# nv-tlabs/vid2player3d

Measured on AMD Instinct MI355X. Metric: env-steps/sec at num_envs=8192, SMPL humanoid imitation, higher is better.
Workload: dtype f32

## Files before the change

vid2player3d_amd/build.py:

```python
import os
import shutil
import subprocess
import sys

HERE = os.path.dirname(os.path.abspath(__file__))
CSRC = os.path.join(HERE, "csrc")
LIB = os.path.join(HERE, "libv2p_rollout.so")
SOURCES = ["capi.hip", "device_owner.hip", "model_compile.hip", "env.hip", "motion_state.hip", "task_ops.hip", "shape_compile.hip", "motion_build.hip", "physics.hip", "physics_ll.hip", "physics_ll_host.hip", "ball_rollout.hip", "tennis_task.hip", "mvae_player.hip", "mvae_player_dual.hip", "mvae_target.hip"]
HEADERS = ["v2p_internal.hpp", "ll_schedule.hpp", "ll_forms.hpp", "v2p_dev.hpp", "v2p_math.inc", "phys_math.hpp", "phys_common.hpp", "motion_sample.inc", "hull_gjk.hpp", "post_ops.inc", "strict_ops.inc", "tennis_task.hpp", "tennis_row.inc", "mvae_player.hpp", "mvae_player_dev.hpp", "mvae_rows.inc", "mvae_target.hpp", os.path.join("..", "..", "include", "v2p_rollout.h")]
ARCH = "gfx950"


def _hipcc():
    for c in (shutil.which("hipcc"), "/opt/rocm/bin/hipcc"):
        if c and os.path.exists(c):
            return c
    raise RuntimeError("hipcc not found: the HIP extension cannot be built")


def needs_build():
    if not os.path.exists(LIB):
        return True
    t = os.path.getmtime(LIB)
    deps = [os.path.join(CSRC, s) for s in SOURCES + HEADERS] + [os.path.abspath(__file__)]
    return any(os.path.getmtime(d) > t for d in deps)


def build_info():
    return {"arch": ARCH, "kernel_source_sha16": kernel_source_hash(), "physics_ll_math": "precise" if os.environ.get("V2P_LL_STRICT_MATH") else "relaxed (" + " ".join(LL_MATH_FLAGS) + "; precise device libraries, strict pre-physics prologue)",
            "hipcc": _hipcc()}


LL_CODEGEN_FLAGS = ["-mllvm", "-sink-insts-to-avoid-spills=1"]
LL_MATH_FLAGS = ["-fassociative-math", "-freciprocal-math", "-fno-signed-zeros", "-fno-trapping-math", "-fno-honor-nans"]
KERNEL_SOURCES = ["physics_ll.hip", "phys_common.hpp", "phys_math.hpp", "hull_gjk.hpp", "strict_ops.inc", "post_ops.inc", "v2p_math.inc", "motion_sample.inc", "v2p_internal.hpp", "ll_schedule.hpp", "ll_forms.hpp", "v2p_dev.hpp"]


def kernel_source_hash():
    import hashlib

    h = hashlib.sha256()
    for s in KERNEL_SOURCES:
        with open(os.path.join(CSRC, s), "rb") as f:
            h.update(s.encode() + b"\0" + f.read() + b"\0")
    h.update(" ".join(LL_MATH_FLAGS + LL_CODEGEN_FLAGS + [os.environ.get("V2P_LL_STRICT_MATH", ""), os.environ.get("V2P_FLAGS_PHYSICS_LL", "")]).encode())
    return h.hexdigest()[:16]


BASE_FLAGS = ["--offload-arch=" + ARCH, "-O3", "-std=c++17", "-fPIC", "-ffp-contract=fast", "-fno-vectorize", "-fno-slp-vectorize", "-Wall",
              "-Wno-unused-function"]
LL_REGS_FLAGS = ["-DV2P_LL_REGS_BUILD", "-DV2P_LL_WPS=2", "-DV2P_LL_WPS_BALL=2", "-DV2P_LL_WPS_LIMITS=2", "-DV2P_LL_PARK2=0", "-DV2P_LL_PARK3=0",
                 "-mllvm", "-amdgpu-sched-strategy=iterative-ilp"]


def compile_flags(source, regs=False):
    fl = list(BASE_FLAGS)
    if regs:
        fl += LL_REGS_FLAGS
    if source in ("motion_state.hip", "task_ops.hip", "shape_compile.hip", "motion_build.hip", "tennis_task.hip", "mvae_player.hip", "mvae_player_dual.hip", "mvae_target.hip"):
        fl = [f if f != "-ffp-contract=fast" else "-ffp-contract=off" for f in fl]
    if source in ("physics_ll.hip", "physics_ll_host.hip", "ball_rollout.hip"):
        fl = [f if f != "-ffp-contract=fast" else "-ffp-contract=fast-honor-pragmas" for f in fl]
        fl = fl + (["-DV2P_LL_STRICT_MATH"] if os.environ.get("V2P_LL_STRICT_MATH") else LL_MATH_FLAGS)
        fl = fl + LL_CODEGEN_FLAGS
    extra = os.environ.get("V2P_FLAGS_" + source.split(".")[0].upper() + ("_REGS" if regs else ""))
    if extra:
        fl = [f for f in fl if f != "-O3"] + extra.split()
    return fl


def build(force=False, verbose=False, lib_out=None, tag=""):
    if lib_out is None and not force and not needs_build():
        return LIB
    objs = []
    procs = []
    for s in SOURCES + ["physics_ll.hip:regs"]:
        regs = s.endswith(":regs")
        s = s.split(":")[0]
        obj = os.path.join(CSRC, s.replace(".hip", ("_regs" if regs else "") + tag + ".o"))
        cmd = [_hipcc()] + compile_flags(s, regs) + ["-c", os.path.join(CSRC, s), "-o", obj]
        if verbose:
            print(" ".join(cmd))
        procs.append((cmd, subprocess.Popen(cmd, stdout=subprocess.PIPE, stderr=subprocess.STDOUT)))
        objs.append(obj)
    for cmd, p in procs:
        out, _ = p.communicate()
        if p.returncode != 0:
            sys.stderr.write(out.decode())
# ... 15 lines not shown
```

vid2player3d_amd/csrc/ll_forms.hpp:

```cpp
#pragma once

namespace v2p {

enum class LlBuild { Lds, Regs };

template <LlBuild BUILD, bool TGS, bool DIAG, bool BALL, bool LIMITS>
struct LlForms {
    static constexpr bool REGS = BUILD == LlBuild::Regs;

    static constexpr bool OPAQUE_H = BALL || LIMITS;

    static constexpr bool FASTARG = REGS ? !BALL && !LIMITS && !TGS && !DIAG
                                         : !BALL && !LIMITS;

    static constexpr bool VTAB = REGS ? !LIMITS && !TGS && !BALL && !DIAG
                                      : !LIMITS && !TGS && !BALL;

    static constexpr bool SETUPX = REGS ? !LIMITS && !TGS && !BALL && !DIAG
                                        : !LIMITS && !TGS && !BALL;

    static constexpr bool LIVEM = VTAB;

    static constexpr bool ROWX = REGS ? VTAB : true;
    static constexpr bool ROWCNT = ROWX && VTAB;

    static constexpr bool UPMASK = !LIMITS && !TGS;

    static constexpr bool LAMX = true;

    static constexpr bool P2SHIFT = !(TGS && BALL);

    static constexpr bool DIAGX = REGS ? false : DIAG;

    static constexpr int waves_per_simd(int wps, int wps_ball, int wps_limits) { return DIAG ? 2 : (BALL ? wps_ball : (LIMITS ? wps_limits : wps)); }

    static_assert(SETUPX == VTAB, "the set-up in front of the sweep and the table go together");
    static_assert(LIVEM == VTAB, "the scalar live word belongs to the visit table");
    static_assert(ROWCNT == (ROWX && VTAB), "the points are counted from the visit words: no table, no count");
    static_assert(!VTAB || UPMASK, "every kernel with the visit table runs the masked way up");
};

}
```

vid2player3d_amd/csrc/physics_ll.hip:

```cpp
#include <hip/hip_runtime.h>
#include <math.h>
#include <stdlib.h>
#include <string.h>

#include <type_traits>

#if !defined(V2P_LL_STRICT_MATH)
#if !defined(V2P_LL_PRECISE_SINCOS)
#define PHYS_SINCOS(x, s, c) do { (s) = __sinf(x); (c) = __cosf(x); } while (0)
#endif
#if !defined(V2P_LL_PRECISE_SQRT)
#define PHYS_SQRT(x) __builtin_amdgcn_sqrtf(x)
#endif
#if !defined(V2P_LL_PRECISE_RCP)
#define PHYS_RCP(x) __builtin_amdgcn_rcpf(x)
#endif
#endif
#include "phys_common.hpp"
#include "hull_gjk.hpp"
#include "ll_forms.hpp"

#if defined(V2P_LL_REGS_BUILD)
#define V2P_LL_NS ll_regs
#define V2P_LL_LAUNCHER launch_env_physics_ll_regs
// ... 125 lines not shown

__device__ __forceinline__ int half_max_last(int v) {
    int o = __builtin_amdgcn_update_dpp(0, v, 0x111, 0xf, 0xf, true); v = o > v ? o : v;
    o = __builtin_amdgcn_update_dpp(0, v, 0x112, 0xf, 0xf, true); v = o > v ? o : v;
    o = __builtin_amdgcn_update_dpp(0, v, 0x114, 0xf, 0xf, true); v = o > v ? o : v;
    o = __builtin_amdgcn_update_dpp(0, v, 0x118, 0xf, 0xf, true); v = o > v ? o : v;
    o = __builtin_amdgcn_update_dpp(0, v, 0x142, 0xa, 0xf, false); v = o > v ? o : v;
    return v;
}

#define LLSAMPLED (((a.prof_heavy ? blockIdx.x < 8u : (blockIdx.x & 63) == 0)) && lane == 0)
#define LLADD(k, v) if (LLSAMPLED) atomicAdd((unsigned long long*)&a.prof[k], (unsigned long long)(v))
#define LLCOUNT(k, v) if (DIAG && a.prof && LLSAMPLED) atomicAdd((unsigned long long*)&a.prof[k], (unsigned long long)(v))
#define LLSUBV(k, tv) do { if (DIAG && a.prof) { long long t_ = clock64(); LLADD(k, t_ - tv); tv = t_; } } while (0)
#define LLSUB(k) LLSUBV(k, tsub)
#define LLSUBX(k, tv) do { if constexpr (F::DIAGX) LLSUBV(k, tv); } while (0)
#define LLSUBX_OR(k, kparent) LLSUB(F::DIAGX ? (k) : (kparent))
#define LLPH(k) LLSUBV(k, tprev)

inline namespace V2P_LL_NS {
#ifndef V2P_LL_WPS
#define V2P_LL_WPS 3
#endif
#ifndef V2P_LL_WPS_BALL
#define V2P_LL_WPS_BALL 3
#endif
#ifndef V2P_LL_WPS_LIMITS
#define V2P_LL_WPS_LIMITS 3
#endif
constexpr int LL_WPB = V2P_LL_WPB;
constexpr LlBuild LL_BUILD = V2P_LL_BUILD;
#ifndef V2P_LL_PARK2
#define V2P_LL_PARK2 1
#endif
constexpr bool PARK2 = V2P_LL_PARK2 != 0;
#ifndef V2P_LL_PARK3
#define V2P_LL_PARK3 1
#endif
constexpr bool PARK3 = V2P_LL_PARK3 != 0;
#ifndef V2P_LL_WAIT_SLEEP
#define V2P_LL_WAIT_SLEEP 16
#endif
constexpr int PARK_TAR = 0, PARK_W0 = 3, PARK_XD0 = 6, PARK_Q = 9, PARK_X = 13, PARK_CR = 16, PARK_CB = 28, PARK_CL = 32,
              PARK_SCR = PARK3 ? 44 : 16,
              PARK_SLOTS = PARK_SCR + 1;
constexpr int ROOTLAM_FLOATS = 2 * 24;
constexpr int BL_POS = 0, BL_QUAT = 3, BL_VEL = 7, BL_ANG = 10, BL_F = 13, BL_GA = 16, BL_GGAP = 17, BL_GBIAS = 18, BL_GLAM = 19, BL_GREST = 22, BL_RK = 24,
              RK_A = 0, RK_GAP = 1, RK_BIAS = 2, RK_RL = 3, RK_N = 6, RK_LAM = 9, RK_LINK = 12, RK_REST = 13, NBREC = 5, BL_V0 = BL_RK + 16 * NBREC, BL_SLOTS = BL_V0 + 8;
constexpr int ROOTLAM_ROW = ROOTLAM_FLOATS / 2, STAGE_FLOATS = NB * 13, REWARD_SLOTS = 4;
constexpr int WRENCH_FORCE_LANE = 0, WRENCH_TORQUE_LANE = 25;
constexpr int LDS_PARK = 0, LDS_STAGE = LDS_PARK, LDS_BALL = LDS_PARK + PARK_SLOTS * 64, LDS_ROOTLAM = LDS_BALL + 2 * BL_SLOTS;
constexpr int LDS_FLOATS_PER_WAVE = LDS_ROOTLAM + ROOTLAM_FLOATS;
static_assert(LDS_STAGE + 2 * STAGE_FLOATS <= LDS_BALL && REWARD_SLOTS <= PARK_SLOTS, "an overlay does not fit the parking slots");
static_assert(WRENCH_TORQUE_LANE > NB && WRENCH_TORQUE_LANE < LPE, "the torque's lane must be one without a link (and not the ball's)");
__device__ __forceinline__ void wrench_put(float* envcol, int l, float x, float y, float z) {
    envcol[l + PARK_TAR * 64] = x; envcol[l + (PARK_TAR + 1) * 64] = y; envcol[l + (PARK_TAR + 2) * 64] = z;
}
__device__ __forceinline__ float wrench_at(const float* envcol, int l, int k) { return envcol[l + (PARK_TAR + k) * 64]; }
__device__ __forceinline__ V3 wrench_get(const float* envcol, int l) { return V3{wrench_at(envcol, l, 0), wrench_at(envcol, l, 1), wrench_at(envcol, l, 2)}; }
__device__ __noinline__ f4 ball_hull_distance(ConstShape* S, int v0, int nv, V3 c) {
    V3 p;
    const float d = hull_closest([&](int k) { return V3{S->hull_verts[v0 + k][0], S->hull_verts[v0 + k][1], S->hull_verts[v0 + k][2]}; }, nv, c, p);
    return f4{p.x, p.y, p.z, d};
}
template <bool LDS>
struct ContactStore;
template <>
struct ContactStore<false> {
    V3 r_[4];
    float b_[4];
    V3 l_[4];
    __device__ __forceinline__ explicit ContactStore(float*) {}
    __device__ __forceinline__ V3 cr(int c) const { return r_[c]; }
    __device__ __forceinline__ void set_cr(int c, V3 v) { r_[c] = v; }
    __device__ __forceinline__ float bias(int c) const { return b_[c]; }
    __device__ __forceinline__ void set_bias(int c, float v) { b_[c] = v; }
    __device__ __forceinline__ V3 lam(int c) const { return l_[c]; }
    __device__ __forceinline__ void set_lam(int c, V3 v) { l_[c] = v; }
};
template <>
struct ContactStore<true> {
    float* p;
    __device__ __forceinline__ explicit ContactStore(float* park) : p(park) {}
    __device__ __forceinline__ V3 cr(int c) const { return V3{p[(PARK_CR + 3 * c) * 64], p[(PARK_CR + 3 * c + 1) * 64], p[(PARK_CR + 3 * c + 2) * 64]}; }
    __device__ __forceinline__ void set_cr(int c, V3 v) { p[(PARK_CR + 3 * c) * 64] = v.x; p[(PARK_CR + 3 * c + 1) * 64] = v.y; p[(PARK_CR + 3 * c + 2) * 64] = v.z; }
    __device__ __forceinline__ float bias(int c) const { return p[(PARK_CB + c) * 64]; }
    __device__ __forceinline__ void set_bias(int c, float v) { p[(PARK_CB + c) * 64] = v; }
    __device__ __forceinline__ V3 lam(int c) const { return V3{p[(PARK_CL + 3 * c) * 64], p[(PARK_CL + 3 * c + 1) * 64], p[(PARK_CL + 3 * c + 2) * 64]}; }
    __device__ __forceinline__ void set_lam(int c, V3 v) { p[(PARK_CL + 3 * c) * 64] = v.x; p[(PARK_CL + 3 * c + 1) * 64] = v.y; p[(PARK_CL + 3 * c + 2) * 64] = v.z; }
};

__device__ __forceinline__ void vfric_frame(const V3& w0, const V3& xd0, const V3& rr, V3& t1, V3& t2) {
    const float vx = xd0.x + w0.y * rr.z - w0.z * rr.y, vy = xd0.y + w0.z * rr.x - w0.x * rr.z;
    const float s2 = vx * vx + vy * vy;
    const bool on = s2 > 1e-12f;
    const float inv = on ? rsqrtf(s2) : 0.f;
    t1 = on ? V3{vx * inv, vy * inv, 0.f} : V3{1.f, 0.f, 0.f};
    t2 = V3{-t1.y, t1.x, 0.f};
}
template <bool CONTACT, bool MULTI, bool TGS, bool DIAG, bool BALL, bool JOBS, bool LIMITS, bool VFRIC = false>
__global__ __launch_bounds__(64 * LL_WPB, (LlForms<LL_BUILD, TGS, DIAG, BALL, LIMITS>::waves_per_simd(V2P_LL_WPS, V2P_LL_WPS_BALL, V2P_LL_WPS_LIMITS))) void physics_ll_kernel(PhysArgs a) {
    using F = LlForms<LL_BUILD, TGS, DIAG, BALL, LIMITS>;
    const int64_t N = a.n;
    const int lane = threadIdx.x & 63;
    const int half = lane >> 5;
    const int lb = lane & (LPE - 1);
// ... 391 lines not shown
                if (valid && !racket_lane) {
                    cb = mulT(R, bp - x);
                    const V3 ac{S->aabb_c[bo][0], S->aabb_c[bo][1], S->aabb_c[bo][2]}, ae{S->aabb_e[bo][0], S->aabb_e[bo][1], S->aabb_e[bo][2]};
                    const V3 ex{fmaxf(fabsf(cb.x - ac.x) - ae.x, 0.f), fmaxf(fabsf(cb.y - ac.y) - ae.y, 0.f), fmaxf(fabsf(cb.z - ac.z) - ae.z, 0.f)};
                    const V3 dv = bv0 - xd;
                    const float vmax = PHYS_SQRT(dot(dv, dv)) + PHYS_SQRT(dot(w, w)) * (PHYS_SQRT(dot(ac, ac)) + PHYS_SQRT(dot(ae, ae)));
                    const float reach = BP.radius + coff + h * vmax;
                    near = dot(ex, ex) < reach * reach && S->hull_count[bo] > 0;
                }
                if (any64(near)) {
                    float gap = 3.0e38f;
                    V3 rlw{0.f, 0.f, 0.f}, nw{0.f, 0.f, 1.f};
                    if (near) {
                        const int hv0 = S->hull_offsets[bo], hnv = S->hull_count[bo];
                        const f4 hc = ball_hull_distance(S, hv0, hnv, cb);
                        V3 pb{hc.x, hc.y, hc.z};
                        float dist = hc.w;
                        V3 nb;
                        if (dist > 1e-6f) nb = PHYS_RCP(dist) * (cb - pb);
                        else {
                            const V3 ev = cb - V3{S->aabb_c[bo][0], S->aabb_c[bo][1], S->aabb_c[bo][2]};
                            const float l = PHYS_SQRT(dot(ev, ev));
                            nb = l > 1e-5f ? PHYS_RCP(l) * ev : V3{0.f, 0.f, 1.f};
                            dist = 0.f;
                            pb = cb;
                        }
                        nw = mul(R, nb);
                        rlw = mul(R, pb);
                        const float vrel = dot(bv0 - xd - cross(w, rlw), nw);
                        const float g = dist - BP.radius;
                        if (g < coff + h * fmaxf(0.f, -vrel)) gap = g;
                    }
#pragma unroll 1
                    for (int k = 0; k < NBREC - 2; ++k) {
                        float gmin = gap;
#pragma unroll
                        for (int sh = 1; sh < 32; sh <<= 1) gmin = fminf(gmin, __shfl_xor(gmin, sh));
                        const unsigned long long wb = __ballot(gap == gmin && gap < 3.0e38f);
                        if (!wb) break;
                        const unsigned wmine = half ? (unsigned)(wb >> 32) : (unsigned)wb;
                        if (wmine && lb == __ffs(wmine) - 1) {
                            lds_vfloat* rk = bl + BL_RK + 16 * (2 + k);
                            rk[RK_A] = 1.f;
                            rk[RK_GAP] = gap;
                            rk[RK_RL] = rlw.x; rk[RK_RL + 1] = rlw.y; rk[RK_RL + 2] = rlw.z;
                            rk[RK_N] = nw.x; rk[RK_N + 1] = nw.y; rk[RK_N + 2] = nw.z;
                            rk[RK_LINK] = (float)lb;
                            gap = 3.0e38f;
                        }
                    }
                }
            }
        }
        const float mass = S->mass[bo];
        const V3 com{S->com[bo][0], S->com[bo][1], S->com[bo][2]};
        const Sym3 Ib{S->inertia[bo][0], S->inertia[bo][1], S->inertia[bo][2], S->inertia[bo][3], S->inertia[bo][4], S->inertia[bo][5]};
        V3 tau{0.f, 0.f, 0.f};
        float lsgn[3] = {0.f, 0.f, 0.f}, lbias[3] = {0.f, 0.f, 0.f}, llam[3] = {0.f, 0.f, 0.f};
        bool limact = false;
        Sym3 Kd{1.f, 0.f, 0.f, 1.f, 0.f, 1.f};
        Sym3 A;
        M3 B;
        Sym3 C{mass, 0.f, 0.f, mass, 0.f, mass};
        V3 pn, pf;
        {
            const M3 R = q2mat(q);
            const float kp = S->kp[bo], kd = S->kd[bo];
            const V3 qe = b != 0 ? quat_to_expmap_stable(jq) : V3{0.f, 0.f, 0.f};
            if (b != 0) tau = mul(R, kp * (park_get3(PARK_TAR) - qe) - (kd + h * kp) * wt);
            if (LIMITS) {
                limact = false;
                const float ih = PHYS_RCP(h);
#pragma unroll
                for (int i = 0; i < 3; ++i) {
                    const float lo = S->limit_lo[bo][i], hi = S->limit_hi[bo][i], qi = i == 0 ? qe.x : (i == 1 ? qe.y : qe.z);
                    const bool on = P.joint_limits && valid && b != 0 && hi - lo < 6.28f;
                    const float clo = qi - lo, chi = hi - qi;
                    const float gap = clo <= chi ? clo : chi;
                    lsgn[i] = on ? (clo <= chi ? 1.f : -1.f) : 0.f;
                    lbias[i] = TGS ? gap : (gap >= 0.f ? gap * ih : fmaxf(P.erp * gap * ih, -P.max_depen));
                    llam[i] = 0.f;
                    limact = limact || on;
                }
            }
            V3 dc = mul(R, com);
            V3 k0 = mul(Ib, V3{R.m[0], R.m[1], R.m[2]});
            V3 k1 = mul(Ib, V3{R.m[3], R.m[4], R.m[5]});
            V3 k2 = mul(Ib, V3{R.m[6], R.m[7], R.m[8]});
            V3 r0 = row(R, 0), r1 = row(R, 1), r2 = row(R, 2);
            Sym3 Ic{dot(r0, k0), dot(r0, k1), dot(r0, k2), dot(r1, k1), dot(r1, k2), dot(r2, k2)};
            float dd = dot(dc, dc);
            A = Sym3{Ic.xx + mass * (dd - dc.x * dc.x), Ic.xy - mass * dc.x * dc.y, Ic.xz - mass * dc.x * dc.z,
                     Ic.yy + mass * (dd - dc.y * dc.y), Ic.yz - mass * dc.y * dc.z, Ic.zz + mass * (dd - dc.z * dc.z)};
            B.m[0] = 0.f;            B.m[1] = -mass * dc.z;  B.m[2] = mass * dc.y;
            B.m[3] = mass * dc.z;    B.m[4] = 0.f;           B.m[5] = -mass * dc.x;
            B.m[6] = -mass * dc.y;   B.m[7] = mass * dc.x;   B.m[8] = 0.f;
            V3 wwd = cross(w, cross(w, dc));
            pf = mass * (wwd - V3{0.f, 0.f, P.gravity_z});
            pn = cross(w, mul(Ic, w)) + cross(dc, pf);
            if (b == 0 && wrench_on) {
                V3 extF, extT;
                if (a.actions) {
                    extF = wrench_get(wrench_park, WRENCH_FORCE_LANE);
                    extT = wrench_get(wrench_park, WRENCH_TORQUE_LANE);
                } else {
                    const float* cw = a.ctrl + env_here() * CTRL_SLOTS;
// ... 82 lines not shown
                }
            }
        }

        LLPH(PROF_PASS2);
        unpark_vel(w, xd);
        Blocks Lam;
        Lam.A = Lam.C = Sym3{1.f, 0.f, 0.f, 1.f, 0.f, 1.f};
#pragma unroll
        for (int i = 0; i < 9; ++i) Lam.B.m[i] = 0.f;
        V3 al{0.f, 0.f, 0.f}, ac{0.f, 0.f, 0.f}, dw{0.f, 0.f, 0.f}, dv{0.f, 0.f, 0.f};
        if (lb == 0) {
            float a6[21], inv6[21];
            a6[tri(0, 0)] = A.xx; a6[tri(1, 0)] = A.xy; a6[tri(2, 0)] = A.xz; a6[tri(1, 1)] = A.yy; a6[tri(2, 1)] = A.yz; a6[tri(2, 2)] = A.zz;
#pragma unroll
            for (int i = 0; i < 3; ++i)
#pragma unroll
                for (int j = 0; j < 3; ++j) a6[tri(3 + i, j)] = B.m[3 * j + i];
            a6[tri(3, 3)] = C.xx; a6[tri(4, 3)] = C.xy; a6[tri(5, 3)] = C.xz; a6[tri(4, 4)] = C.yy; a6[tri(5, 4)] = C.yz; a6[tri(5, 5)] = C.zz;
            spd6_inverse(a6, inv6);
            Lam.A = Sym3{inv6[tri(0, 0)], inv6[tri(1, 0)], inv6[tri(2, 0)], inv6[tri(1, 1)], inv6[tri(2, 1)], inv6[tri(2, 2)]};
#pragma unroll
            for (int i = 0; i < 3; ++i)
#pragma unroll
                for (int j = 0; j < 3; ++j) Lam.B.m[3 * i + j] = inv6[tri(3 + j, i)];
            Lam.C = Sym3{inv6[tri(3, 3)], inv6[tri(4, 3)], inv6[tri(5, 3)], inv6[tri(4, 4)], inv6[tri(5, 4)], inv6[tri(5, 5)]};
            al = -(mul(Lam.A, pn) + mul(Lam.B, pf));
            ac = -(V3{dot(col(Lam.B, 0), pn), dot(col(Lam.B, 1), pn), dot(col(Lam.B, 2), pn)} + mul(Lam.C, pf));
            dw = h * al;
            dv = h * ac;
            w = w + dw;
            xd = xd + dv;
        }

        for (int d = 1; d <= maxd; ++d) {
            const bool nc = (nonchain >> d) & 1;
            V3 alp = pp(al, nc), acp = pp(ac, nc), dwp = pp(dw, nc), dvp = pp(dv, nc);
            if (dep == d) {
                V3 aw = alp + zw;
                V3 av = acp + cross(alp, r) + zv;
                V3 qdd = mul(Di, u + aug * aw) - aw - mul(E, av);
                al = aw + qdd;
                ac = av;
                dw = dwp + h * qdd;
                dv = dvp + cross(dwp, r);
                w = w + dw;
                xd = xd + dv;
            }
        }

        LLPH(PROF_PASS3);
        if (CONTACT) park_vel(w, xd);
        float* const rootlam = wave_lds + LDS_ROOTLAM + half * ROOTLAM_ROW;
        if (PARK2 && CONTACT && lb == 0) {
            const float lv[21] = {Lam.A.xx, Lam.A.xy, Lam.A.xz, Lam.A.yy, Lam.A.yz, Lam.A.zz, Lam.B.m[0], Lam.B.m[1], Lam.B.m[2], Lam.B.m[3], Lam.B.m[4], Lam.B.m[5],
                                  Lam.B.m[6], Lam.B.m[7], Lam.B.m[8], Lam.C.xx, Lam.C.xy, Lam.C.xz, Lam.C.yy, Lam.C.yz, Lam.C.zz};
#pragma unroll
            for (int k = 0; k < 21; ++k) rootlam[k] = lv[k];
        }
        if (PARK2 && CONTACT) {
            Lam.A = Lam.C = Sym3{1.f, 0.f, 0.f, 1.f, 0.f, 1.f};
#pragma unroll
            for (int i = 0; i < 9; ++i) Lam.B.m[i] = 0.f;
        }
        q = Q4{park[PARK_Q * 64], park[(PARK_Q + 1) * 64], park[(PARK_Q + 2) * 64], park[(PARK_Q + 3) * 64]};
        x = park_get3(PARK_X);
        int cnt = 0;
        ContactStore<PARK3> CS(park);
#pragma unroll
        for (int c = 0; c < 4; ++c) { CS.set_cr(c, V3{0.f, 0.f, 0.f}); CS.set_bias(c, 0.f); CS.set_lam(c, V3{0.f, 0.f, 0.f}); }
        if (CONTACT) {
            const float coff = P.contact_offset;
            const int v0 = S->hull_offsets[bo], nv = S->hull_count[bo];
            const float rz0 = 2.f * (q.x * q.z - q.w * q.y), rz1 = 2.f * (q.y * q.z + q.w * q.x), rz2 = 1.f - 2.f * (q.x * q.x + q.y * q.y);
            const float zlow = x.z + rz0 * S->aabb_c[bo][0] + rz1 * S->aabb_c[bo][1] + rz2 * S->aabb_c[bo][2] -
                               (fabsf(rz0) * S->aabb_e[bo][0] + fabsf(rz1) * S->aabb_e[bo][1] + fabsf(rz2) * S->aabb_e[bo][2]);
            const bool near = valid && (zlow < coff + 1e-4f);
            int pack = 0x0fffffff;
            long long tsub = DIAG && a.prof ? clock64() : 0;
            const unsigned long long nball = __ballot(near);
            LLSUB(PROF_CULL);
            if (nball) {
                const unsigned nm = half ? (unsigned)(nball >> 32) : (unsigned)nball;
                const int nr0 = __popc((unsigned)nball), nr1 = __popc((unsigned)(nball >> 32));
                const int ntot = nr0 + nr1;
                const int rounds = (ntot + 7) >> 3;
                const int myk = (half ? nr0 : 0) + __popc(nm & ((1u << lb) - 1u));
                const int grp = lane >> 3, gl = lane & 7;
                int* const scr = (int*)(wave_lds + LDS_PARK + PARK_SCR * 64);
                if (near) scr[myk] = lane;
                LLCOUNT(PROF_ROUNDS, rounds);
                for (int rd = 0; rd < rounds; ++rd) {
                    const int kk = 8 * rd + grp;
                    const bool gon = kk < ntot;
                    const int src = gon ? scr[kk] : lane;
                    const M3 RL = q2mat(pull(q, src));
                    const V3 xL = pull(x, src);
                    const float r6 = RL.m[6], r7 = RL.m[7], r8 = RL.m[8], xz = xL.z;
                    const int v0L = __builtin_amdgcn_ds_bpermute(src << 2, v0), nvL = __builtin_amdgcn_ds_bpermute(src << 2, nv);
                    ConstShape* const SL = MULTI ? (ConstShape*)(a.shapes + __builtin_amdgcn_ds_bpermute(src << 2, sid)) : S;
                    auto hullv = [&](int idx) -> float4 { return make_float4(SL->hull_verts[idx][0], SL->hull_verts[idx][1], SL->hull_verts[idx][2], 0.f); };
                    const float r0 = RL.m[0], r1 = RL.m[1], r2 = RL.m[2], xx = xL.x;
                    const float r3 = RL.m[3], r4 = RL.m[4], r5 = RL.m[5], xy = xL.y;
                    const unsigned gbit = 1u << gl;
                    float4 vv[8];
#pragma unroll
                    for (int k = 0; k < 8; ++k) {
                        const int i = 8 * k + gl;
                        vv[k] = hullv(v0L + ((gon && i < nvL) ? i : 0));
                    }
                    float px[8], py[8];
                    unsigned clo = 0u, chi = 0u;
                    int k0 = -1;
                    float zmin = 0.f;
#pragma unroll
                    for (int k = 0; k < 8; ++k) {
                        const int i = 8 * k + gl;
                        const bool in = gon && i < nvL;
                        const float z = xz + r6 * vv[k].x + r7 * vv[k].y + r8 * vv[k].z;
                        px[k] = xx + r0 * vv[k].x + r1 * vv[k].y + r2 * vv[k].z;
                        py[k] = xy + r3 * vv[k].x + r4 * vv[k].y + r5 * vv[k].z;
                        const bool c = in && (z < coff);
                        const unsigned bit = c ? gbit << (8 * (k & 3)) : 0u;
                        if (k < 4) clo |= bit; else chi |= bit;
                        const bool better = c && (k0 < 0 || z < zmin);
                        k0 = better ? i : k0;
                        zmin = better ? z : zmin;
                    }
                    clo |= grp_xor1(clo); chi |= grp_xor1(chi);
                    clo |= grp_xor2(clo); chi |= grp_xor2(chi);
                    clo |= grp_mirror(clo); chi |= grp_mirror(chi);
                    grp_arg<false, F::FASTARG>(zmin, k0);
                    const unsigned long long cm = ((unsigned long long)chi << 32) | clo;
                    const int cntg = __popc(clo) + __popc(chi);
                    unsigned long long t = cm;
                    int s0 = t ? __ffsll((long long)t) - 1 : -1; t &= t - 1;
                    int s1 = t ? __ffsll((long long)t) - 1 : -1; t &= t - 1;
                    int s2 = t ? __ffsll((long long)t) - 1 : -1; t &= t - 1;
                    int s3 = t ? __ffsll((long long)t) - 1 : -1;
                    int ns = cntg < 4 ? cntg : 4;
                    const bool big = gon && cntg > 4;
                    if (any64(big)) {
                        LLCOUNT(PROF_MANIFOLDS, 1ull);
                        const int k0s = k0 < 0 ? 0 : k0;
                        const float4 u0 = hullv(v0L + k0s);
                        const float p0x = xx + r0 * u0.x + r1 * u0.y + r2 * u0.z;
                        const float p0y = xy + r3 * u0.x + r4 * u0.y + r5 * u0.z;
                        const unsigned long long remB = big ? (cm & ~(1ull << k0s)) : 0ull;
                        const unsigned blo = (unsigned)remB, bhi = (unsigned)(remB >> 32);
                        int k1 = -1;
                        float best = -1.f;
#pragma unroll
                        for (int k = 0; k < 8; ++k) {
                            const bool on = ((k < 4 ? blo : bhi) & (gbit << (8 * (k & 3)))) != 0u;
                            const float dx = px[k] - p0x, dy = py[k] - p0y;
                            const float d2 = dx * dx + dy * dy;
                            const bool take = on && (d2 > best);
                            best = take ? d2 : best;
                            k1 = take ? 8 * k + gl : k1;
                        }
                        grp_arg<true, F::FASTARG>(best, k1);
                        const int k1s = k1 < 0 ? 0 : k1;
                        const float4 u1 = hullv(v0L + k1s);
                        const float ex = xx + r0 * u1.x + r1 * u1.y + r2 * u1.z - p0x;
                        const float ey = xy + r3 * u1.x + r4 * u1.y + r5 * u1.z - p0y;
                        const unsigned long long remC = remB & ~(1ull << k1s);
                        const unsigned elo = (unsigned)remC, ehi = (unsigned)(remC >> 32);
                        int k2 = -1, k3 = -1;
                        float amax = 0.f, amin = 0.f;
#pragma unroll
                        for (int k = 0; k < 8; ++k) {
                            const bool on = ((k < 4 ? elo : ehi) & (gbit << (8 * (k & 3)))) != 0u;
                            const float dx = px[k] - p0x, dy = py[k] - p0y;
                            const float area = ex * dy - ey * dx;
                            const bool up = on && area > amax;
                            const bool dn = on && area < amin;
                            amax = up ? area : amax; k2 = up ? 8 * k + gl : k2;
                            amin = dn ? area : amin; k3 = dn ? 8 * k + gl : k3;
                        }
                        grp_arg<true, F::FASTARG>(amax, k2);
                        grp_arg<false, F::FASTARG>(amin, k3);
                        if (big) {
                            s0 = k0; s1 = k1;
                            s2 = k2 >= 0 ? k2 : k3;
                            s3 = k2 >= 0 ? k3 : -1;
                            ns = 2 + (k2 >= 0 ? 1 : 0) + (k3 >= 0 ? 1 : 0);
                        }
                    }
                    const int gpack = (s0 & 0x7f) | ((s1 & 0x7f) << 7) | ((s2 & 0x7f) << 14) | ((s3 & 0x7f) << 21) | (ns << 28);
                    const int got = __builtin_amdgcn_ds_bpermute(((myk & 7) << 3) << 2, gpack);
                    pack = (near && (myk >> 3) == rd) ? got : pack;
                }
            }
            LLSUB(PROF_SCAN);
            int sel4[4];
#pragma unroll
            for (int c = 0; c < 4; ++c) {
                const int sv = (pack >> (7 * c)) & 0x7f;
                sel4[c] = sv == 0x7f ? -1 : sv;
            }
            cnt = (pack >> 28) & 7;
            if (any64(cnt > 0)) {
                const M3 R = q2mat(q);
                const float ih = 1.f / h;
#pragma unroll
                for (int c = 0; c < 4; ++c) {
                    const float4 uu = hullv(v0 + (sel4[c] < 0 ? 0 : sel4[c]));
                    const V3 crc = mul(R, V3{uu.x, uu.y, uu.z});
                    CS.set_cr(c, crc);
                    float dz = x.z + crc.z - P.rest_offset;
                    CS.set_bias(c, TGS ? dz : (dz >= 0.f ? dz * ih : fmaxf(P.erp * dz * ih, -P.max_depen)));
                }
            }
            if (a.contact_ids && last && valid && live_env && !frozen) {
#pragma unroll
                for (int c = 0; c < 4; ++c) a.contact_ids[(env_here() * NB + b) * 4 + c] = c < cnt ? b * 64 + sel4[c] : -1;
            }
            if (a.contact_ids_sub && valid && live_env && !frozen) {
#pragma unroll
                for (int c = 0; c < 4; ++c) a.contact_ids_sub[((env_here() * nsub + sub) * NB + b) * 4 + c] = c < cnt ? b * 64 + sel4[c] : -1;
            }

            LLSUB(PROF_POINTS);
            if (PARK2 && lb == 0) {
                float lv[21];
#pragma unroll
                for (int k = 0; k < 21; ++k) lv[k] = rootlam[k];
                Lam.A = Sym3{lv[0], lv[1], lv[2], lv[3], lv[4], lv[5]};
#pragma unroll
                for (int k = 0; k < 9; ++k) Lam.B.m[k] = lv[6 + k];
                Lam.C = Sym3{lv[15], lv[16], lv[17], lv[18], lv[19], lv[20]};
            }
            auto ball_rec_mine = [&](int j) -> bool { return j < 2 ? racket_lane : lb == (int)bl[BL_RK + 16 * j + RK_LINK]; };
            bool myhull = false;
            if (BALL) {
#pragma unroll
                for (int j = 2; j < NBREC; ++j) myhull = myhull || (bl[BL_RK + 16 * j + RK_A] != 0.f && lb == (int)bl[BL_RK + 16 * j + RK_LINK]);
            }
            const bool ballhit = BALL && valid && ((racket_lane && (bl[BL_RK + RK_A] != 0.f || bl[BL_RK + 16 + RK_A] != 0.f)) || myhull);
            const bool ballground = BALL && ball_lane && bl[BL_GA] != 0.f;
            const bool touched = valid && (cnt > 0 || ballhit);
            const unsigned long long tb = __ballot(touched);
            const unsigned m0 = (unsigned)tb, m1 = (unsigned)(tb >> 32);
            if (LIMITS && any64(limact)) {
                const V3 wv = PARK2 ? park_get3(PARK_W0) : w;
                const V3 pwv = pp(wv, true);
                const V3 om = mulT(q2mat(q), wv - pwv);
                const float mrate = P.limit_margin * PHYS_RCP(h);
                const float lscale = TGS ? PHYS_RCP(h) : 1.f;
                bool anyrow = false;
#pragma unroll
                for (int i = 0; i < 3; ++i) {
                    const float omi = i == 0 ? om.x : (i == 1 ? om.y : om.z);
                    const bool on = lsgn[i] != 0.f && lbias[i] * lscale < mrate + fmaxf(0.f, -lsgn[i] * omi);
                    if (!on) lsgn[i] = 0.f;
                    anyrow = anyrow || on;
                }
                limact = anyrow;
            }
            const unsigned long long lmb = LIMITS ? __ballot(valid && limact) : 0ull;
            const unsigned lm0 = (unsigned)lmb, lm1 = (unsigned)(lmb >> 32);
            if (DIAG && a.wave_times) { const int tt = __popc(half ? m1 : m0); tsum += tt; tmaxs = tt > tmaxs ? tt : tmaxs; }
            [[maybe_unused]] int tdep0 = 0, tdep1 = 0;
            if constexpr (F::SETUPX) {
                const int tdred = half_max_last(touched ? dep : 0);
                tdep0 = __builtin_amdgcn_readlane(tdred, 31);
                tdep1 = __builtin_amdgcn_readlane(tdred, 63);
            }
            if (last) {
                const unsigned mine = half ? m1 : m0;
                ksum = __popc(mine);
                if constexpr (F::SETUPX) {
                    kdep = half ? tdep1 : tdep0;
                } else {
                    kdep = 0;
                    for (unsigned t = mine; t; t &= t - 1) { const int dd = M.depth[__ffs(t) - 1]; kdep = dd > kdep ? dd : kdep; }
                }
// ... 1052 lines not shown
```

Measured before the change: 23.89 million.

## Generate contacts before the articulated passes in visit-table kernels

Moves contact generation (hull culling, vertex scan, manifold selection) into a shared include and, for kernel forms that use the visit table, runs it right after the pose is known instead of after pass 3. This avoids parking and reloading q, x and the root Lambda through LDS around the contact scan. It also shifts register pressure, since the contact store is now live across the mass-matrix passes. A static assert is added to check that the parking slots used by the passes do not overlap the contact records or the scratch row.

```diff
diff --git a/vid2player3d_amd/build.py b/vid2player3d_amd/build.py
--- a/vid2player3d_amd/build.py
+++ b/vid2player3d_amd/build.py
@@ -7,7 +7,7 @@
 CSRC = os.path.join(HERE, "csrc")
 LIB = os.path.join(HERE, "libv2p_rollout.so")
 SOURCES = ["capi.hip", "device_owner.hip", "model_compile.hip", "env.hip", "motion_state.hip", "task_ops.hip", "shape_compile.hip", "motion_build.hip", "physics.hip", "physics_ll.hip", "physics_ll_host.hip", "ball_rollout.hip", "tennis_task.hip", "mvae_player.hip", "mvae_player_dual.hip", "mvae_target.hip"]
-HEADERS = ["v2p_internal.hpp", "ll_schedule.hpp", "ll_forms.hpp", "v2p_dev.hpp", "v2p_math.inc", "phys_math.hpp", "phys_common.hpp", "motion_sample.inc", "hull_gjk.hpp", "post_ops.inc", "strict_ops.inc", "tennis_task.hpp", "tennis_row.inc", "mvae_player.hpp", "mvae_player_dev.hpp", "mvae_rows.inc", "mvae_target.hpp", os.path.join("..", "..", "include", "v2p_rollout.h")]
+HEADERS = ["v2p_internal.hpp", "ll_schedule.hpp", "ll_forms.hpp", "ll_contact_setup.inc", "v2p_dev.hpp", "v2p_math.inc", "phys_math.hpp", "phys_common.hpp", "motion_sample.inc", "hull_gjk.hpp", "post_ops.inc", "strict_ops.inc", "tennis_task.hpp", "tennis_row.inc", "mvae_player.hpp", "mvae_player_dev.hpp", "mvae_rows.inc", "mvae_target.hpp", os.path.join("..", "..", "include", "v2p_rollout.h")]
 ARCH = "gfx950"
 
 
@@ -33,7 +33,7 @@
 
 LL_CODEGEN_FLAGS = ["-mllvm", "-sink-insts-to-avoid-spills=1"]
 LL_MATH_FLAGS = ["-fassociative-math", "-freciprocal-math", "-fno-signed-zeros", "-fno-trapping-math", "-fno-honor-nans"]
-KERNEL_SOURCES = ["physics_ll.hip", "phys_common.hpp", "phys_math.hpp", "hull_gjk.hpp", "strict_ops.inc", "post_ops.inc", "v2p_math.inc", "motion_sample.inc", "v2p_internal.hpp", "ll_schedule.hpp", "ll_forms.hpp", "v2p_dev.hpp"]
+KERNEL_SOURCES = ["physics_ll.hip", "phys_common.hpp", "phys_math.hpp", "hull_gjk.hpp", "strict_ops.inc", "post_ops.inc", "v2p_math.inc", "motion_sample.inc", "v2p_internal.hpp", "ll_schedule.hpp", "ll_forms.hpp", "ll_contact_setup.inc", "v2p_dev.hpp"]
 
 
 def kernel_source_hash():
diff --git a/vid2player3d_amd/csrc/ll_contact_setup.inc b/vid2player3d_amd/csrc/ll_contact_setup.inc
--- /dev/null
+++ b/vid2player3d_amd/csrc/ll_contact_setup.inc
@@ -0,0 +1,156 @@
+#pragma unroll
+for (int c = 0; c < 4; ++c) { CS.set_cr(c, V3{0.f, 0.f, 0.f}); CS.set_bias(c, 0.f); CS.set_lam(c, V3{0.f, 0.f, 0.f}); }
+if (CONTACT) {
+    const float coff = P.contact_offset;
+    const int v0 = S->hull_offsets[bo], nv = S->hull_count[bo];
+    const float rz0 = 2.f * (q.x * q.z - q.w * q.y), rz1 = 2.f * (q.y * q.z + q.w * q.x), rz2 = 1.f - 2.f * (q.x * q.x + q.y * q.y);
+    const float zlow = x.z + rz0 * S->aabb_c[bo][0] + rz1 * S->aabb_c[bo][1] + rz2 * S->aabb_c[bo][2] -
+                       (fabsf(rz0) * S->aabb_e[bo][0] + fabsf(rz1) * S->aabb_e[bo][1] + fabsf(rz2) * S->aabb_e[bo][2]);
+    const bool near = valid && (zlow < coff + 1e-4f);
+    int pack = 0x0fffffff;
+    long long tsub = DIAG && a.prof ? clock64() : 0;
+    const unsigned long long nball = __ballot(near);
+    LLSUB(PROF_CULL);
+    if (nball) {
+        const unsigned nm = half ? (unsigned)(nball >> 32) : (unsigned)nball;
+        const int nr0 = __popc((unsigned)nball), nr1 = __popc((unsigned)(nball >> 32));
+        const int ntot = nr0 + nr1;
+        const int rounds = (ntot + 7) >> 3;
+        const int myk = (half ? nr0 : 0) + __popc(nm & ((1u << lb) - 1u));
+        const int grp = lane >> 3, gl = lane & 7;
+        int* const scr = (int*)(wave_lds + LDS_PARK + PARK_SCR * 64);
+        if (near) scr[myk] = lane;
+        LLCOUNT(PROF_ROUNDS, rounds);
+        for (int rd = 0; rd < rounds; ++rd) {
+            const int kk = 8 * rd + grp;
+            const bool gon = kk < ntot;
+            const int src = gon ? scr[kk] : lane;
+            const M3 RL = q2mat(pull(q, src));
+            const V3 xL = pull(x, src);
+            const float r6 = RL.m[6], r7 = RL.m[7], r8 = RL.m[8], xz = xL.z;
+            const int v0L = __builtin_amdgcn_ds_bpermute(src << 2, v0), nvL = __builtin_amdgcn_ds_bpermute(src << 2, nv);
+            ConstShape* const SL = MULTI ? (ConstShape*)(a.shapes + __builtin_amdgcn_ds_bpermute(src << 2, sid)) : S;
+            auto hullv = [&](int idx) -> float4 { return make_float4(SL->hull_verts[idx][0], SL->hull_verts[idx][1], SL->hull_verts[idx][2], 0.f); };
+            const float r0 = RL.m[0], r1 = RL.m[1], r2 = RL.m[2], xx = xL.x;
+            const float r3 = RL.m[3], r4 = RL.m[4], r5 = RL.m[5], xy = xL.y;
+            const unsigned gbit = 1u << gl;
+            float4 vv[8];
+#pragma unroll
+            for (int k = 0; k < 8; ++k) {
+                const int i = 8 * k + gl;
+                vv[k] = hullv(v0L + ((gon && i < nvL) ? i : 0));
+            }
+            float px[8], py[8];
+            unsigned clo = 0u, chi = 0u;
+            int k0 = -1;
+            float zmin = 0.f;
+#pragma unroll
+            for (int k = 0; k < 8; ++k) {
+                const int i = 8 * k + gl;
+                const bool in = gon && i < nvL;
+                const float z = xz + r6 * vv[k].x + r7 * vv[k].y + r8 * vv[k].z;
+                px[k] = xx + r0 * vv[k].x + r1 * vv[k].y + r2 * vv[k].z;
+                py[k] = xy + r3 * vv[k].x + r4 * vv[k].y + r5 * vv[k].z;
+                const bool c = in && (z < coff);
+                const unsigned bit = c ? gbit << (8 * (k & 3)) : 0u;
+                if (k < 4) clo |= bit; else chi |= bit;
+                const bool better = c && (k0 < 0 || z < zmin);
+                k0 = better ? i : k0;
+                zmin = better ? z : zmin;
+            }
+            clo |= grp_xor1(clo); chi |= grp_xor1(chi);
+            clo |= grp_xor2(clo); chi |= grp_xor2(chi);
+            clo |= grp_mirror(clo); chi |= grp_mirror(chi);
+            grp_arg<false, F::FASTARG>(zmin, k0);
+            const unsigned long long cm = ((unsigned long long)chi << 32) | clo;
+            const int cntg = __popc(clo) + __popc(chi);
+            unsigned long long t = cm;
+            int s0 = t ? __ffsll((long long)t) - 1 : -1; t &= t - 1;
+            int s1 = t ? __ffsll((long long)t) - 1 : -1; t &= t - 1;
+            int s2 = t ? __ffsll((long long)t) - 1 : -1; t &= t - 1;
+            int s3 = t ? __ffsll((long long)t) - 1 : -1;
+            int ns = cntg < 4 ? cntg : 4;
+            const bool big = gon && cntg > 4;
+            if (any64(big)) {
+                LLCOUNT(PROF_MANIFOLDS, 1ull);
+                const int k0s = k0 < 0 ? 0 : k0;
+                const float4 u0 = hullv(v0L + k0s);
+                const float p0x = xx + r0 * u0.x + r1 * u0.y + r2 * u0.z;
+                const float p0y = xy + r3 * u0.x + r4 * u0.y + r5 * u0.z;
+                const unsigned long long remB = big ? (cm & ~(1ull << k0s)) : 0ull;
+                const unsigned blo = (unsigned)remB, bhi = (unsigned)(remB >> 32);
+                int k1 = -1;
+                float best = -1.f;
+#pragma unroll
+                for (int k = 0; k < 8; ++k) {
+                    const bool on = ((k < 4 ? blo : bhi) & (gbit << (8 * (k & 3)))) != 0u;
+                    const float dx = px[k] - p0x, dy = py[k] - p0y;
+                    const float d2 = dx * dx + dy * dy;
+                    const bool take = on && (d2 > best);
+                    best = take ? d2 : best;
+                    k1 = take ? 8 * k + gl : k1;
+                }
+                grp_arg<true, F::FASTARG>(best, k1);
+                const int k1s = k1 < 0 ? 0 : k1;
+                const float4 u1 = hullv(v0L + k1s);
+                const float ex = xx + r0 * u1.x + r1 * u1.y + r2 * u1.z - p0x;
+                const float ey = xy + r3 * u1.x + r4 * u1.y + r5 * u1.z - p0y;
+                const unsigned long long remC = remB & ~(1ull << k1s);
+                const unsigned elo = (unsigned)remC, ehi = (unsigned)(remC >> 32);
+                int k2 = -1, k3 = -1;
+                float amax = 0.f, amin = 0.f;
+#pragma unroll
+                for (int k = 0; k < 8; ++k) {
+                    const bool on = ((k < 4 ? elo : ehi) & (gbit << (8 * (k & 3)))) != 0u;
+                    const float dx = px[k] - p0x, dy = py[k] - p0y;
+                    const float area = ex * dy - ey * dx;
+                    const bool up = on && area > amax;
+                    const bool dn = on && area < amin;
+                    amax = up ? area : amax; k2 = up ? 8 * k + gl : k2;
+                    amin = dn ? area : amin; k3 = dn ? 8 * k + gl : k3;
+                }
+                grp_arg<true, F::FASTARG>(amax, k2);
+                grp_arg<false, F::FASTARG>(amin, k3);
+                if (big) {
+                    s0 = k0; s1 = k1;
+                    s2 = k2 >= 0 ? k2 : k3;
+                    s3 = k2 >= 0 ? k3 : -1;
+                    ns = 2 + (k2 >= 0 ? 1 : 0) + (k3 >= 0 ? 1 : 0);
+                }
+            }
+            const int gpack = (s0 & 0x7f) | ((s1 & 0x7f) << 7) | ((s2 & 0x7f) << 14) | ((s3 & 0x7f) << 21) | (ns << 28);
+            const int got = __builtin_amdgcn_ds_bpermute(((myk & 7) << 3) << 2, gpack);
+            pack = (near && (myk >> 3) == rd) ? got : pack;
+        }
+    }
+    LLSUB(PROF_SCAN);
+    int sel4[4];
+#pragma unroll
+    for (int c = 0; c < 4; ++c) {
+        const int sv = (pack >> (7 * c)) & 0x7f;
+        sel4[c] = sv == 0x7f ? -1 : sv;
+    }
+    cnt = (pack >> 28) & 7;
+    if (any64(cnt > 0)) {
+        const M3 R = q2mat(q);
+        const float ih = 1.f / h;
+#pragma unroll
+        for (int c = 0; c < 4; ++c) {
+            const float4 uu = hullv(v0 + (sel4[c] < 0 ? 0 : sel4[c]));
+            const V3 crc = mul(R, V3{uu.x, uu.y, uu.z});
+            CS.set_cr(c, crc);
+            float dz = x.z + crc.z - P.rest_offset;
+            CS.set_bias(c, TGS ? dz : (dz >= 0.f ? dz * ih : fmaxf(P.erp * dz * ih, -P.max_depen)));
+        }
+    }
+    if (a.contact_ids && last && valid && live_env && !frozen) {
+#pragma unroll
+        for (int c = 0; c < 4; ++c) a.contact_ids[(env_here() * NB + b) * 4 + c] = c < cnt ? b * 64 + sel4[c] : -1;
+    }
+    if (a.contact_ids_sub && valid && live_env && !frozen) {
+#pragma unroll
+        for (int c = 0; c < 4; ++c) a.contact_ids_sub[((env_here() * nsub + sub) * NB + b) * 4 + c] = c < cnt ? b * 64 + sel4[c] : -1;
+    }
+
+    LLSUB(PROF_POINTS);
+}
diff --git a/vid2player3d_amd/csrc/ll_forms.hpp b/vid2player3d_amd/csrc/ll_forms.hpp
--- a/vid2player3d_amd/csrc/ll_forms.hpp
+++ b/vid2player3d_amd/csrc/ll_forms.hpp
@@ -30,6 +30,8 @@
 
     static constexpr bool P2SHIFT = !(TGS && BALL);
 
+    static constexpr bool CGEN_EARLY = VTAB;
+
     static constexpr bool DIAGX = REGS ? false : DIAG;
 
     static constexpr int waves_per_simd(int wps, int wps_ball, int wps_limits) { return DIAG ? 2 : (BALL ? wps_ball : (LIMITS ? wps_limits : wps)); }
diff --git a/vid2player3d_amd/csrc/physics_ll.hip b/vid2player3d_amd/csrc/physics_ll.hip
--- a/vid2player3d_amd/csrc/physics_ll.hip
+++ b/vid2player3d_amd/csrc/physics_ll.hip
@@ -201,6 +201,9 @@
 constexpr int LDS_PARK = 0, LDS_STAGE = LDS_PARK, LDS_BALL = LDS_PARK + PARK_SLOTS * 64, LDS_ROOTLAM = LDS_BALL + 2 * BL_SLOTS;
 constexpr int LDS_FLOATS_PER_WAVE = LDS_ROOTLAM + ROOTLAM_FLOATS;
 static_assert(LDS_STAGE + 2 * STAGE_FLOATS <= LDS_BALL && REWARD_SLOTS <= PARK_SLOTS, "an overlay does not fit the parking slots");
+static_assert(PARK_TAR + 3 <= PARK_W0 && PARK_W0 + 3 <= PARK_XD0 && PARK_XD0 + 3 <= PARK_Q && PARK_Q + 4 <= PARK_X && PARK_X + 3 <= PARK_CR && PARK_X + 3 <= PARK_SCR &&
+                  (!PARK3 || (PARK_CR + 12 <= PARK_CB && PARK_CB + 4 <= PARK_CL && PARK_CL + 12 <= PARK_SCR)),
+              "a pass's parking slots overlap the contact records or the scratch row");
 static_assert(WRENCH_TORQUE_LANE > NB && WRENCH_TORQUE_LANE < LPE, "the torque's lane must be one without a link (and not the ball's)");
 __device__ __forceinline__ void wrench_put(float* envcol, int l, float x, float y, float z) {
     envcol[l + PARK_TAR * 64] = x; envcol[l + (PARK_TAR + 1) * 64] = y; envcol[l + (PARK_TAR + 2) * 64] = z;
@@ -698,6 +701,17 @@
                 }
             }
         }
+        [[maybe_unused]] int cnt_early = 0;
+        [[maybe_unused]] ContactStore<PARK3> CS_early(park);
+        if constexpr (F::CGEN_EARLY) {
+            LLPH(PROF_PASS1);
+            int cnt = 0;
+            ContactStore<PARK3> CS(park);
+#include "ll_contact_setup.inc"
+            cnt_early = cnt;
+            CS_early = CS;
+            LLPH(PROF_CONTACTS);
+        }
         const float mass = S->mass[bo];
         const V3 com{S->com[bo][0], S->com[bo][1], S->com[bo][2]};
         const Sym3 Ib{S->inertia[bo][0], S->inertia[bo][1], S->inertia[bo][2], S->inertia[bo][3], S->inertia[bo][4], S->inertia[bo][5]};
@@ -886,177 +900,31 @@
         LLPH(PROF_PASS3);
         if (CONTACT) park_vel(w, xd);
         float* const rootlam = wave_lds + LDS_ROOTLAM + half * ROOTLAM_ROW;
-        if (PARK2 && CONTACT && lb == 0) {
+        if (PARK2 && CONTACT && !F::CGEN_EARLY && lb == 0) {
             const float lv[21] = {Lam.A.xx, Lam.A.xy, Lam.A.xz, Lam.A.yy, Lam.A.yz, Lam.A.zz, Lam.B.m[0], Lam.B.m[1], Lam.B.m[2], Lam.B.m[3], Lam.B.m[4], Lam.B.m[5],
                                   Lam.B.m[6], Lam.B.m[7], Lam.B.m[8], Lam.C.xx, Lam.C.xy, Lam.C.xz, Lam.C.yy, Lam.C.yz, Lam.C.zz};
 #pragma unroll
             for (int k = 0; k < 21; ++k) rootlam[k] = lv[k];
         }
-        if (PARK2 && CONTACT) {
+        if (PARK2 && CONTACT && !F::CGEN_EARLY) {
             Lam.A = Lam.C = Sym3{1.f, 0.f, 0.f, 1.f, 0.f, 1.f};
 #pragma unroll
             for (int i = 0; i < 9; ++i) Lam.B.m[i] = 0.f;
         }
-        q = Q4{park[PARK_Q * 64], park[(PARK_Q + 1) * 64], park[(PARK_Q + 2) * 64], park[(PARK_Q + 3) * 64]};
-        x = park_get3(PARK_X);
+        if constexpr (!F::CGEN_EARLY) {
+            q = Q4{park[PARK_Q * 64], park[(PARK_Q + 1) * 64], park[(PARK_Q + 2) * 64], park[(PARK_Q + 3) * 64]};
+            x = park_get3(PARK_X);
+        }
         int cnt = 0;
         ContactStore<PARK3> CS(park);
-#pragma unroll
-        for (int c = 0; c < 4; ++c) { CS.set_cr(c, V3{0.f, 0.f, 0.f}); CS.set_bias(c, 0.f); CS.set_lam(c, V3{0.f, 0.f, 0.f}); }
+        if constexpr (F::CGEN_EARLY) {
+            cnt = cnt_early;
+            CS = CS_early;
+        } else {
+#include "ll_contact_setup.inc"
+        }
         if (CONTACT) {
-            const float coff = P.contact_offset;
-            const int v0 = S->hull_offsets[bo], nv = S->hull_count[bo];
-            const float rz0 = 2.f * (q.x * q.z - q.w * q.y), rz1 = 2.f * (q.y * q.z + q.w * q.x), rz2 = 1.f - 2.f * (q.x * q.x + q.y * q.y);
-            const float zlow = x.z + rz0 * S->aabb_c[bo][0] + rz1 * S->aabb_c[bo][1] + rz2 * S->aabb_c[bo][2] -
-                               (fabsf(rz0) * S->aabb_e[bo][0] + fabsf(rz1) * S->aabb_e[bo][1] + fabsf(rz2) * S->aabb_e[bo][2]);
-            const bool near = valid && (zlow < coff + 1e-4f);
-            int pack = 0x0fffffff;
-            long long tsub = DIAG && a.prof ? clock64() : 0;
-            const unsigned long long nball = __ballot(near);
-            LLSUB(PROF_CULL);
-            if (nball) {
-                const unsigned nm = half ? (unsigned)(nball >> 32) : (unsigned)nball;
-                const int nr0 = __popc((unsigned)nball), nr1 = __popc((unsigned)(nball >> 32));
-                const int ntot = nr0 + nr1;
-                const int rounds = (ntot + 7) >> 3;
-                const int myk = (half ? nr0 : 0) + __popc(nm & ((1u << lb) - 1u));
-                const int grp = lane >> 3, gl = lane & 7;
-                int* const scr = (int*)(wave_lds + LDS_PARK + PARK_SCR * 64);
-                if (near) scr[myk] = lane;
-                LLCOUNT(PROF_ROUNDS, rounds);
-                for (int rd = 0; rd < rounds; ++rd) {
-                    const int kk = 8 * rd + grp;
-                    const bool gon = kk < ntot;
-                    const int src = gon ? scr[kk] : lane;
-                    const M3 RL = q2mat(pull(q, src));
-                    const V3 xL = pull(x, src);
-                    const float r6 = RL.m[6], r7 = RL.m[7], r8 = RL.m[8], xz = xL.z;
-                    const int v0L = __builtin_amdgcn_ds_bpermute(src << 2, v0), nvL = __builtin_amdgcn_ds_bpermute(src << 2, nv);
-                    ConstShape* const SL = MULTI ? (ConstShape*)(a.shapes + __builtin_amdgcn_ds_bpermute(src << 2, sid)) : S;
-                    auto hullv = [&](int idx) -> float4 { return make_float4(SL->hull_verts[idx][0], SL->hull_verts[idx][1], SL->hull_verts[idx][2], 0.f); };
-                    const float r0 = RL.m[0], r1 = RL.m[1], r2 = RL.m[2], xx = xL.x;
-                    const float r3 = RL.m[3], r4 = RL.m[4], r5 = RL.m[5], xy = xL.y;
-                    const unsigned gbit = 1u << gl;
-                    float4 vv[8];
-#pragma unroll
-                    for (int k = 0; k < 8; ++k) {
-                        const int i = 8 * k + gl;
-                        vv[k] = hullv(v0L + ((gon && i < nvL) ? i : 0));
-                    }
-                    float px[8], py[8];
-                    unsigned clo = 0u, chi = 0u;
-                    int k0 = -1;
-                    float zmin = 0.f;
-#pragma unroll
-                    for (int k = 0; k < 8; ++k) {
-                        const int i = 8 * k + gl;
-                        const bool in = gon && i < nvL;
-                        const float z = xz + r6 * vv[k].x + r7 * vv[k].y + r8 * vv[k].z;
-                        px[k] = xx + r0 * vv[k].x + r1 * vv[k].y + r2 * vv[k].z;
-                        py[k] = xy + r3 * vv[k].x + r4 * vv[k].y + r5 * vv[k].z;
-                        const bool c = in && (z < coff);
-                        const unsigned bit = c ? gbit << (8 * (k & 3)) : 0u;
-                        if (k < 4) clo |= bit; else chi |= bit;
-                        const bool better = c && (k0 < 0 || z < zmin);
-                        k0 = better ? i : k0;
-                        zmin = better ? z : zmin;
-                    }
-                    clo |= grp_xor1(clo); chi |= grp_xor1(chi);
-                    clo |= grp_xor2(clo); chi |= grp_xor2(chi);
-                    clo |= grp_mirror(clo); chi |= grp_mirror(chi);
-                    grp_arg<false, F::FASTARG>(zmin, k0);
-                    const unsigned long long cm = ((unsigned long long)chi << 32) | clo;
-                    const int cntg = __popc(clo) + __popc(chi);
-                    unsigned long long t = cm;
-                    int s0 = t ? __ffsll((long long)t) - 1 : -1; t &= t - 1;
-                    int s1 = t ? __ffsll((long long)t) - 1 : -1; t &= t - 1;
-                    int s2 = t ? __ffsll((long long)t) - 1 : -1; t &= t - 1;
-                    int s3 = t ? __ffsll((long long)t) - 1 : -1;
-                    int ns = cntg < 4 ? cntg : 4;
-                    const bool big = gon && cntg > 4;
-                    if (any64(big)) {
-                        LLCOUNT(PROF_MANIFOLDS, 1ull);
-                        const int k0s = k0 < 0 ? 0 : k0;
-                        const float4 u0 = hullv(v0L + k0s);
-                        const float p0x = xx + r0 * u0.x + r1 * u0.y + r2 * u0.z;
-                        const float p0y = xy + r3 * u0.x + r4 * u0.y + r5 * u0.z;
-                        const unsigned long long remB = big ? (cm & ~(1ull << k0s)) : 0ull;
-                        const unsigned blo = (unsigned)remB, bhi = (unsigned)(remB >> 32);
-                        int k1 = -1;
-                        float best = -1.f;
-#pragma unroll
-                        for (int k = 0; k < 8; ++k) {
-                            const bool on = ((k < 4 ? blo : bhi) & (gbit << (8 * (k & 3)))) != 0u;
-                            const float dx = px[k] - p0x, dy = py[k] - p0y;
-                            const float d2 = dx * dx + dy * dy;
-                            const bool take = on && (d2 > best);
-                            best = take ? d2 : best;
-                            k1 = take ? 8 * k + gl : k1;
-                        }
-                        grp_arg<true, F::FASTARG>(best, k1);
-                        const int k1s = k1 < 0 ? 0 : k1;
-                        const float4 u1 = hullv(v0L + k1s);
-                        const float ex = xx + r0 * u1.x + r1 * u1.y + r2 * u1.z - p0x;
-                        const float ey = xy + r3 * u1.x + r4 * u1.y + r5 * u1.z - p0y;
-                        const unsigned long long remC = remB & ~(1ull << k1s);
-                        const unsigned elo = (unsigned)remC, ehi = (unsigned)(remC >> 32);
-                        int k2 = -1, k3 = -1;
-                        float amax = 0.f, amin = 0.f;
-#pragma unroll
-                        for (int k = 0; k < 8; ++k) {
-                            const bool on = ((k < 4 ? elo : ehi) & (gbit << (8 * (k & 3)))) != 0u;
-                            const float dx = px[k] - p0x, dy = py[k] - p0y;
-                            const float area = ex * dy - ey * dx;
-                            const bool up = on && area > amax;
-                            const bool dn = on && area < amin;
-                            amax = up ? area : amax; k2 = up ? 8 * k + gl : k2;
-                            amin = dn ? area : amin; k3 = dn ? 8 * k + gl : k3;
-                        }
-                        grp_arg<true, F::FASTARG>(amax, k2);
-                        grp_arg<false, F::FASTARG>(amin, k3);
-                        if (big) {
-                            s0 = k0; s1 = k1;
-                            s2 = k2 >= 0 ? k2 : k3;
-                            s3 = k2 >= 0 ? k3 : -1;
-                            ns = 2 + (k2 >= 0 ? 1 : 0) + (k3 >= 0 ? 1 : 0);
-                        }
-                    }
-                    const int gpack = (s0 & 0x7f) | ((s1 & 0x7f) << 7) | ((s2 & 0x7f) << 14) | ((s3 & 0x7f) << 21) | (ns << 28);
-                    const int got = __builtin_amdgcn_ds_bpermute(((myk & 7) << 3) << 2, gpack);
-                    pack = (near && (myk >> 3) == rd) ? got : pack;
-                }
-            }
-            LLSUB(PROF_SCAN);
-            int sel4[4];
-#pragma unroll
-            for (int c = 0; c < 4; ++c) {
-                const int sv = (pack >> (7 * c)) & 0x7f;
-                sel4[c] = sv == 0x7f ? -1 : sv;
-            }
-            cnt = (pack >> 28) & 7;
-            if (any64(cnt > 0)) {
-                const M3 R = q2mat(q);
-                const float ih = 1.f / h;
-#pragma unroll
-                for (int c = 0; c < 4; ++c) {
-                    const float4 uu = hullv(v0 + (sel4[c] < 0 ? 0 : sel4[c]));
-                    const V3 crc = mul(R, V3{uu.x, uu.y, uu.z});
-                    CS.set_cr(c, crc);
-                    float dz = x.z + crc.z - P.rest_offset;
-                    CS.set_bias(c, TGS ? dz : (dz >= 0.f ? dz * ih : fmaxf(P.erp * dz * ih, -P.max_depen)));
-                }
-            }
-            if (a.contact_ids && last && valid && live_env && !frozen) {
-#pragma unroll
-                for (int c = 0; c < 4; ++c) a.contact_ids[(env_here() * NB + b) * 4 + c] = c < cnt ? b * 64 + sel4[c] : -1;
-            }
-            if (a.contact_ids_sub && valid && live_env && !frozen) {
-#pragma unroll
-                for (int c = 0; c < 4; ++c) a.contact_ids_sub[((env_here() * nsub + sub) * NB + b) * 4 + c] = c < cnt ? b * 64 + sel4[c] : -1;
-            }
-
-            LLSUB(PROF_POINTS);
-            if (PARK2 && lb == 0) {
+            if (PARK2 && !F::CGEN_EARLY && lb == 0) {
                 float lv[21];
 #pragma unroll
                 for (int k = 0; k < 21; ++k) lv[k] = rootlam[k];
```

Measured after the change: 24.15 million, median of 6. +1.1%, better.
